# lvjiahui/DRT

Measured on AMD Instinct MI355X. Metric: M camera-rays/s (forward+backward) on 50k-tri mesh, 72 views, higher is better.
Workload: dtype f32 traversal + f64 shading/gradients; 1 GPU; horse_vh.ply x4 (1 midpoint subdivision) = 50248 tris / 25126 verts, 72 turntable views, 1024x1024 rays/view, LBVH rebuilt every step, forward+ray_loss+backward+all-reduce+SGD; targets=horse_scan.ply, mode=dropin, hip_graph=False, outputs_recycled=True, ray_binding=True, views_per_gpu=72, views_per_call=72

## Files before the change

### drt_amd/_lib.py

```python
from __future__ import annotations

import ctypes
import os

_HERE = os.path.dirname(os.path.abspath(__file__))
LIB_PATH = os.environ.get("DRT_HIP_LIB") or os.path.join(_HERE, "libdrt_hip.so")

_c = ctypes
_P = _c.c_void_p
_I64 = _c.c_int64
_D = _c.c_double

SIGNATURES = {
    "drt_last_error": (_c.c_char_p, []),
    "drt_version": (_c.c_int, []),
    "drt_deterministic": (_c.c_int, [_c.c_int]),
    "drt_fx_finalize": (_c.c_int, [_P, _I64, _P, _c.c_int, _P]),
    "drt_fx_add": (_c.c_int, [_P, _P, _I64, _P]),
    "drt_fx_to_limbs": (_c.c_int, [_P, _I64, _P, _P]),
    "drt_fx_from_limbs": (_c.c_int, [_P, _I64, _P, _P]),
    "drt_create": (_c.c_int, [_c.c_int, _c.POINTER(_P)]),
    "drt_destroy": (None, [_P]),
    "drt_update_mesh": (_c.c_int, [_P, _P, _I64, _P, _I64, _P]),
    "drt_update_vert": (_c.c_int, [_P, _P, _I64, _P]),
# ... 76 lines not shown
    "drt_rm_split_faces": (_c.c_int, [_P, _I64, _P, _P, _P, _P, _P]),
    "drt_rm_vertex_normals": (_c.c_int, [_P, _P, _P, _P, _I64, _P, _P]),
    "drt_rm_vertex_faces": (_c.c_int, [_P, _I64, _I64, _P, _P, _P, _P, _P, _P, _P]),
    "drt_rm_collapse_eval_all": (_c.c_int, [_P, _I64, _P, _P, _P, _P, _D, _D, _c.c_int, _P, _P, _P, _P, _P, _P, _P, _P, _I64, _P, _P]),
    "drt_rm_surface_filter_list": (_c.c_int, [_P, _P, _P, _P, _P, _I64, _D, _P, _P]),
    "drt_rm_surface_filter": (_c.c_int, [_P, _P, _P, _P, _I64, _c.c_int, _D, _P, _P]),
    "drt_rm_closest_near": (_c.c_int, [_P, _P, _I64, _D, _P, _P]),
    "drt_rm_kill_faces": (_c.c_int, [_P, _P, _I64, _P, _P]),
    "drt_rm_collapse_apply": (_c.c_int, [_P, _I64, _P, _P, _P, _P, _P, _P, _I64, _D, _c.c_uint32, _c.c_int, _P, _P, _P, _P, _P, _c.c_int, _P, _P, _P]),
    "drt_rm_round_end": (_c.c_int, [_P, _c.c_int, _P]),
    "drt_rm_flip_eval": (_c.c_int, [_P, _I64, _P, _P, _P, _P, _D, _P, _P, _P, _P, _P]),
    "drt_rm_flip_apply": (_c.c_int, [_I64, _P, _P, _P, _I64, _c.c_int, _P, _P, _c.c_int, _P, _P, _P]),
    "drt_rm_smooth_target": (_c.c_int, [_P, _P, _P, _P, _I64, _P, _P]),
    "drt_rm_face_agreement": (_c.c_int, [_P, _P, _P, _I64, _P, _P]),
    "drt_rm_move_check": (_c.c_int, [_P, _P, _P, _P, _P, _I64, _I64, _P, _P, _P]),
    "drt_mesh_buf_size": (_c.c_int, [_P, _c.POINTER(_I64), _c.POINTER(_I64), _P]),
    "drt_mesh_buf_copy": (_c.c_int, [_P, _P, _P]),
    "drt_mesh_buf_free": (None, [_P]),
    "drt_profile_enable": (_c.c_int, [_P, _c.c_int]),
    "drt_profile_select": (_c.c_int, [_P, _c.c_uint32]),
    "drt_profile_read": (_c.c_int, [_P, _P, _P, _P]),
    "drt_profile_trace_stats": (_c.c_int, [_P, _P]),
    "drt_route_counts": (_c.c_int, [_P, _P]),
    "drt_check_violations": (_c.c_int, [_P]),
}

_lib = None


class DrtError(RuntimeError):
    pass


def lib():
    global _lib
    if _lib is None:
        if not os.path.exists(LIB_PATH):
            raise DrtError(f"{LIB_PATH} not found: the HIP extension is not built "
                           "(run `python __graft_entry__.py`); there is no CPU fallback")
        h = ctypes.CDLL(LIB_PATH)
        for name, (res, args) in SIGNATURES.items():
            if os.environ.get("DRT_HIP_LIB") and not hasattr(h, name):
                continue
            fn = getattr(h, name)
            fn.restype = res
            fn.argtypes = args
# ... 12 lines not shown
```

### drt_amd/csrc/drt_api.hip

```cpp
#include "drt_scene.h"

static thread_local char g_err[512] = "";
int fail(int code, const char* fmt, ...) {
    va_list ap;
    va_start(ap, fmt);
    vsnprintf(g_err, sizeof(g_err), fmt, ap);
    va_end(ap);
    return code;
}

int ensure_slow_stack(drt_scene* s, hipStream_t st) {
    if (s->slow_stack) return DRT_OK;
    hipStreamCaptureStatus cap = hipStreamCaptureStatusNone;
    if (hipStreamIsCapturing(st, &cap) == hipSuccess && cap != hipStreamCaptureStatusNone)
        return fail(DRT_E_INVALID, "the first silhouette / closest-point / intersect query of a scene allocates its overflow area and cannot run inside a "
                                   "stream capture: issue one such call eagerly before capturing");
    int blocks = s->grid_trace;
    if (blocks < 4 * s->n_cu) blocks = 4 * s->n_cu;
    if (blocks < kRedoGrid) blocks = kRedoGrid;
    HIP_TRY(hipMalloc(&s->slow_stack, sizeof(int32_t) * (size_t)blocks * kTraceBlock * kStackSlowDev));
    return DRT_OK;
}

static int g_det = -1;
// ... 94 lines not shown
    if (e == hipSuccess) {
        const uint32_t init[12] = {0xFF800000u, 0xFF800000u, 0xFF800000u, 0x007FFFFFu, 0x007FFFFFu, 0x007FFFFFu,
                                   0xFF800000u, 0xFF800000u, 0xFF800000u, 0x007FFFFFu, 0x007FFFFFu, 0x007FFFFFu};
        e = hipMemcpy(s->bounds_acc, init, sizeof(init), hipMemcpyHostToDevice);
    }
    if (e == hipSuccess) e = hipMalloc(&s->vcount, sizeof(unsigned) * 4);
    if (e == hipSuccess) e = hipMemset(s->vcount, 0, sizeof(unsigned) * 4);
    if (e == hipSuccess) e = hipMalloc(&s->seg_counts, sizeof(unsigned) * drt_scene::kMaxSeg);
    if (e == hipSuccess) e = hipEventCreateWithFlags(&s->fork_ev, hipEventDisableTiming);
    if (e == hipSuccess) e = hipStreamCreateWithFlags(&s->build_stream, hipStreamNonBlocking);
    if (e == hipSuccess) e = hipEventCreateWithFlags(&s->prefill_fork, hipEventDisableTiming);
    if (e == hipSuccess) e = hipEventCreateWithFlags(&s->prefill_done, hipEventDisableTiming);
    if (e == hipSuccess) e = hipEventCreateWithFlags(&s->prefill_done_cap, hipEventDisableTiming);
    if (e == hipSuccess) e = hipEventCreateWithFlags(&s->build_fork, hipEventDisableTiming);
    if (e == hipSuccess) e = hipEventCreateWithFlags(&s->build_done, hipEventDisableTiming);
    if (const char* ev = getenv("DRT_ASYNC_BUILD")) s->async_build = atoi(ev) != 0;
    if (const char* ev = getenv("DRT_CULL_DIRECT")) s->cull_direct = atoi(ev) != 0;
    if (const char* ev = getenv("DRT_CULL_PARK")) s->cull_park = atoi(ev) != 0;
    if (const char* ev = getenv("DRT_CULL_DIRECT_MIN_LOG2")) { const int v = atoi(ev); if (v >= 0 && v <= 40) s->cull_direct_min_rays = (int64_t)1 << v; }
    if (const char* ev = getenv("DRT_TREE")) { const int v = atoi(ev); if (v >= 0 && v <= 2) s->tree_mode = v; }
    if (const char* ev = getenv("DRT_REBUILD_EVERY")) { const int v = atoi(ev); if (v >= 1) s->rebuild_every = v; }
    if (const char* ev = getenv("DRT_STREAMS")) { const int v = atoi(ev); if (v >= 1 && v <= drt_scene::kMaxSub) s->n_sub = v; }
    if (const char* ev = getenv("DRT_RASTER")) s->use_raster = atoi(ev) != 0;
    if (const char* ev = getenv("DRT_HIT_SEED")) s->hit_seed = atoi(ev) != 0;
    if (const char* ev = getenv("DRT_ARM_FINISH_BESIDE")) s->arm_finish_beside = atoi(ev) != 0;
    if (const char* ev = getenv("DRT_SEED_TILED")) s->seed_tiled = atoi(ev) != 0;
    if (const char* ev = getenv("DRT_GRID_CANARY")) s->grid_canary = atoi(ev) != 0;
    if (const char* ev = getenv("DRT_FILL_OVERLAP")) s->fill_overlap = atoi(ev) != 0;
    if (const char* ev = getenv("DRT_FILL_AFTER_SHADE1")) s->fill_after_shade1 = atoi(ev) != 0;
    if (const char* ev = getenv("DRT_SUB_PER_STREAM")) { const int v = atoi(ev); if (v >= 1 && v <= 16) s->sub_per_stream = v; }
    if (const char* ev = getenv("DRT_MIN_SUB_LOG2")) { const int v = atoi(ev); if (v >= 12 && v <= 30) s->min_sub_rays = (int64_t)1 << v; }
    for (int k = 0; k < s->n_sub && e == hipSuccess; ++k) {
        drt_scene::Sub& w = s->sub[k];
        e = hipStreamCreateWithFlags(&w.stream, hipStreamNonBlocking);
        if (e == hipSuccess) e = hipEventCreateWithFlags(&w.done, hipEventDisableTiming);
        if (e == hipSuccess) e = hipEventCreateWithFlags(&w.tail, hipEventDisableTiming);
        if (e == hipSuccess) e = hipEventCreateWithFlags(&w.fill_fork, hipEventDisableTiming);
        if (e == hipSuccess) e = hipEventCreateWithFlags(&w.fill_join, hipEventDisableTiming);
        if (e == hipSuccess) e = hipMalloc(&w.qcount, sizeof(unsigned) * kQCount);
        if (e == hipSuccess) e = hipMalloc(&w.slow_stack, sizeof(int32_t) * (size_t)kRedoGrid * kTraceBlock * kStackSlowDev);
    }
    if (e == hipSuccess) {
        hipDeviceProp_t prop;
        if (hipGetDeviceProperties(&prop, device) == hipSuccess && prop.multiProcessorCount > 0) s->n_cu = prop.multiProcessorCount;
        int per_cu;
        per_cu = query_blocks_per_cu();
// ... 18 lines not shown
        return fail(DRT_E_HIP, "hipMalloc: %s", hipGetErrorString(e));
    }
    *out = s;
    return DRT_OK;
}

void drt_destroy(drt_scene_t* s) {
    if (!s) return;
    (void)hipSetDevice(s->device);
    if (s->build_stream) (void)hipStreamSynchronize(s->build_stream);
    scene_free_mesh(s);
    if (s->build_fork) (void)hipEventDestroy(s->build_fork);
    if (s->build_done) (void)hipEventDestroy(s->build_done);
    if (s->build_stream) (void)hipStreamDestroy(s->build_stream);
    (void)hipFree(s->params);
    (void)hipFree(s->slow_stack);
    (void)hipFree(s->scratch); (void)hipFree(s->bounds_acc); (void)hipFree(s->seg_counts);
    (void)hipFree(s->b1_list); (void)hipFree(s->b1_redo); (void)hipFree(s->b1_count);
    for (int j = 0; j < drt_scene::kMaxSub; ++j) {
        drt_scene::Sub& w = s->sub[j];
        for (int k = 0; k < 3; ++k) { (void)hipFree(w.q_idx[k]); (void)hipFree(w.q_ray[k]); (void)hipFree(w.q_face[k]); }
        (void)hipFree(w.tmp_face1); (void)hipFree(w.tmp_face2); (void)hipFree(w.qcount); (void)hipFree(w.slow_stack); (void)hipFree(w.redo);
        (void)hipFree(w.zbuf); (void)hipFree(w.zmask); (void)hipFree(w.vmodel); (void)hipFree(w.big); (void)hipFree(w.big_count); (void)hipFree(w.gen_list); (void)hipFree(w.ray64);
        if (w.done) (void)hipEventDestroy(w.done);
        if (w.fill_fork) (void)hipEventDestroy(w.fill_fork);
        if (w.fill_join) (void)hipEventDestroy(w.fill_join);
        if (w.tail) (void)hipEventDestroy(w.tail);
        if (w.stream) (void)hipStreamDestroy(w.stream);
    }
    image_views_free(s);
    image_loss_free(s);
    paths_free(s);
    (void)hipFree(s->vcount);
    (void)hipFree(s->vh_list);
    if (s->fork_ev) (void)hipEventDestroy(s->fork_ev);
    if (s->prefill_fork) (void)hipEventDestroy(s->prefill_fork);
    if (s->prefill_done) (void)hipEventDestroy(s->prefill_done);
    if (s->prefill_done_cap) (void)hipEventDestroy(s->prefill_done_cap);
    for (auto& e : s->prof_ev) (void)hipEventDestroy(e);
    (void)hipFree(s->prof_counts);
    delete s;
}

int drt_profile_enable(drt_scene_t* s, int on) {
    CHECK_SCENE(s);
    if (on && s->prof_ev.empty()) {
// ... 30 lines not shown
    for (size_t k = 0; k + 1 < s->prof_used; k += 2) {
        float ms = 0.f;
        HIP_TRY(hipEventElapsedTime(&ms, s->prof_ev[k], s->prof_ev[k + 1]));
        const int stg = s->prof_stage[k / 2];
        ms_out[stg] += ms;
        launches_out[stg] += 1;
    }
    unsigned long long h[kProfStages + 12];
    HIP_TRY(hipMemcpy(h, s->prof_counts, sizeof(h), hipMemcpyDeviceToHost));
    for (int k = 0; k < kProfStages; ++k) items_out[k] = (int64_t)h[k];
    for (int k = 0; k < 12; ++k) s->trace_stats[k] = (int64_t)h[kProfStages + k];
    HIP_TRY(hipMemset(s->prof_counts, 0, sizeof(h)));
    s->prof_used = 0;
    return DRT_OK;
}

int drt_route_counts(drt_scene_t* s, int64_t* out8) {
    CHECK_SCENE(s);
    if (!out8) return fail(DRT_E_INVALID, "null pointer argument");
    for (int k = 0; k < 8; ++k) out8[k] = s->route_counts[k];
    return DRT_OK;
}

int drt_internal_stream(drt_scene_t* s, int which, void** out) {
    if (!s || !out) return fail(DRT_E_INVALID, "null pointer argument");
    if (which == 0) { *out = (void*)s->build_stream; return DRT_OK; }
    if (which >= 1 && which <= s->n_sub) { *out = (void*)s->sub[which - 1].stream; return DRT_OK; }
    return fail(DRT_E_INVALID, "no internal stream %d (0 = build, 1..%d = pipelines)", which, s->n_sub);
}

int drt_check_violations(int64_t* out4) {
    if (!out4) return fail(DRT_E_INVALID, "null pointer argument");
#if defined(DRT_CHECK)
    HIP_TRY(hipDeviceSynchronize());
    unsigned long long tot[4] = {0, 0, 0, 0};
    if (check_counters_pipeline(tot) || check_counters_trace(tot)) return fail(DRT_E_HIP, "could not read the check counters");
    for (int k = 0; k < 4; ++k) out4[k] = (int64_t)tot[k];
#else
    for (int k = 0; k < 4; ++k) out4[k] = -1;
#endif
    return DRT_OK;
}

int drt_profile_trace_stats(drt_scene_t* s, int64_t* out12) {
    CHECK_SCENE(s);
    if (!out12) return fail(DRT_E_INVALID, "null pointer argument");
// ... 7 lines not shown
```

### drt_amd/csrc/drt_build.hip

```cpp
#include "drt_device.h"
#include "drt_sort.h"
#include <algorithm>

void scene_free_mesh(drt_scene* s) {
    (void)hipFree(s->faces); (void)hipFree(s->verts); (void)hipFree(s->nodes); (void)hipFree(s->tris);
    (void)hipFree(s->keys[0]); (void)hipFree(s->keys[1]); (void)hipFree(s->idx[0]); (void)hipFree(s->idx[1]);
    (void)hipFree(s->hist); (void)hipFree(s->parent_inner); (void)hipFree(s->parent_leaf); (void)hipFree(s->flags);
    (void)hipFree(s->wide); (void)hipFree(s->range_lo); (void)hipFree(s->range_hi); (void)hipFree(s->tris_flat); (void)hipFree(s->slot_of_face);
    s->slot_of_face = nullptr; s->wide = nullptr; s->range_lo = s->range_hi = nullptr; s->tris_flat = nullptr;
    s->faces = nullptr; s->verts = nullptr; s->nodes = nullptr; s->tris = nullptr;
    s->keys[0] = s->keys[1] = s->idx[0] = s->idx[1] = nullptr;
    s->hist = nullptr; s->parent_inner = s->parent_leaf = nullptr; s->flags = nullptr;
    s->cap_faces = s->cap_verts = 0;
}

__device__ __forceinline__ uint32_t f32_ordered(float f) { const uint32_t b = __float_as_uint(f); return b ^ ((b >> 31) ? 0xFFFFFFFFu : 0x80000000u); }
__device__ __forceinline__ float f32_unordered(uint32_t u) { return __uint_as_float(u ^ ((u >> 31) ? 0x80000000u : 0xFFFFFFFFu)); }
constexpr uint32_t kOrdPosInf = 0xFF800000u, kOrdNegInf = 0x007FFFFFu;

__global__ void __launch_bounds__(256) k_cast_verts(const double* __restrict__ v64, float* __restrict__ v32, int64_t n3, uint32_t* acc,
                                                    uint32_t* __restrict__ hist_zero, int hist_entries) {
    __shared__ float red[6][4];
    for (int64_t i = blockIdx.x * (int64_t)blockDim.x + threadIdx.x; i < hist_entries; i += (int64_t)gridDim.x * blockDim.x) hist_zero[i] = 0u;
    float lo[3] = {INFINITY, INFINITY, INFINITY}, hi[3] = {-INFINITY, -INFINITY, -INFINITY};
// ... 555 lines not shown
    return DRT_OK;
}

int wait_build(drt_scene* s, hipStream_t st) {
    if (s->build_pending) HIP_TRY(hipStreamWaitEvent(st, s->build_done, 0));
    return DRT_OK;
}

extern "C" {

int drt_update_mesh(drt_scene_t* s, const int32_t* d_faces, int64_t n_faces, const float* d_verts, int64_t n_verts, void* stream) {
    CHECK_SCENE(s);
    if (n_faces < 0 || n_verts < 0 || (n_faces && !d_faces) || (n_verts && !d_verts)) return fail(DRT_E_INVALID, "bad mesh arguments");
    if (n_faces > (int64_t)1 << 30) return fail(DRT_E_INVALID, "too many faces");
    hipStream_t st = (hipStream_t)stream;
    int rc = begin_update(s, st);
    if (rc) return rc;
    if (n_faces > s->cap_faces || n_verts > s->cap_verts) HIP_TRY(hipStreamSynchronize(s->build_stream));
    rc = ensure_capacity(s, n_faces, n_verts);
    if (rc) return rc;
    s->n_faces = n_faces;
    s->n_verts = n_verts;
    s->order_valid = false;
    if (n_faces) HIP_TRY(hipMemcpyAsync(s->faces, d_faces, sizeof(int32_t) * 3 * n_faces, hipMemcpyDeviceToDevice, st));
    if (n_verts) HIP_TRY(hipMemcpyAsync(s->verts, d_verts, sizeof(float) * 3 * n_verts, hipMemcpyDeviceToDevice, st));
    s->topology_fixed = false;
    if (s->tree_mode == 2) { rc = install_sah_topology(s, st); if (rc) return rc; }
    return rebuild(s, st, nullptr);
}

int drt_update_vert(drt_scene_t* s, const float* d_verts, int64_t n_verts, void* stream) {
    CHECK_BUILT(s);
    if (n_verts != s->n_verts || (n_verts && !d_verts)) return fail(DRT_E_INVALID, "vertex count %lld != %lld", (long long)n_verts, (long long)s->n_verts);
    hipStream_t st = (hipStream_t)stream;
    int rc = begin_update(s, st);
    if (rc) return rc;
    if (n_verts) HIP_TRY(hipMemcpyAsync(s->verts, d_verts, sizeof(float) * 3 * n_verts, hipMemcpyDeviceToDevice, st));
    return rebuild(s, st, nullptr);
}

int drt_update_vert_f64(drt_scene_t* s, const double* d_verts, int64_t n_verts, void* stream) {
    CHECK_BUILT(s);
    if (n_verts != s->n_verts || (n_verts && !d_verts)) return fail(DRT_E_INVALID, "vertex count %lld != %lld", (long long)n_verts, (long long)s->n_verts);
    hipStream_t st = (hipStream_t)stream;
    int rc = begin_update(s, st);
    if (rc) return rc;
// ... 62 lines not shown
```

### drt_amd/csrc/drt_raster.h

```cpp
#pragma once
#include "drt_common.h"
#include "drt_tri.h"

namespace drt {

struct ViewModel {
    double o[3];
    double minv[9];
    int32_t ok;
    int32_t all;
};

static_assert(sizeof(ViewModel) == 104, "DRT_GRID_CACHE_BYTES of include/drt_hip.h");

constexpr double kRasterPad = 0.0625;
constexpr double kRasterVerifyTol = 1e-3;
#ifndef DRT_RASTER_MAX_PER_LANE
#define DRT_RASTER_MAX_PER_LANE 48
#endif
constexpr int kRasterMaxPerLane = DRT_RASTER_MAX_PER_LANE;
constexpr int kRasterBandPixels = 1024;

DRT_HD bool fit_view_model(d3 o, d3 d00, d3 dW0, d3 d0H, d3 dWH, double wm1, double hm1, ViewModel& vm) {
    const d3 c0 = dW0, c1 = d0H, c2 = -dWH;
// ... 52 lines not shown
    const float fx0 = fmaxf(ceilf(lox), 0.0f), fx1 = fminf(floorf(hix), (float)(w - 1));
    const float fy0 = fmaxf(ceilf(loy), 0.0f), fy1 = fminf(floorf(hiy), (float)(h - 1));
    if (fx0 > fx1 || fy0 > fy1) return r;
    r.x0 = (int)fx0; r.x1 = (int)fx1; r.y0 = (int)fy0; r.y1 = (int)fy1;
    return r;
}

DRT_HD bool tri_faces_away(f3 o32, const TriRec& t) {
    const f3 a{t.v0x - o32.x, t.v0y - o32.y, t.v0z - o32.z};
    return dot(a, cross(f3{t.e1x, t.e1y, t.e1z}, f3{t.e2x, t.e2y, t.e2z})) > 0.0f;
}

DRT_HD unsigned long long raster_key(float t, int32_t face) {
    uint32_t tb;
    memcpy(&tb, &t, 4);
    return ((unsigned long long)tb << 32) | (unsigned long long)(uint32_t)face;
}
constexpr unsigned long long kRasterEmpty = ~0ull;

DRT_HD int64_t raster_slot(unsigned x, unsigned gy, unsigned w) {
    return (((int64_t)(gy >> 2) * (w >> 2) + (x >> 2)) << 4) | ((gy & 3u) << 2) | (x & 3u);
}

}
```

### drt_amd/csrc/drt_raster.hip

```cpp
#include "drt_device.h"

__global__ void __launch_bounds__(64) k_fit_views(const double* __restrict__ origin, const double* __restrict__ dir, int w, int h,
                                                  ViewModel* __restrict__ views) {
    __shared__ ViewModel vm;
    const int64_t base = (int64_t)blockIdx.x * w * h;
    if (threadIdx.x == 0) {
        const int64_t i00 = base, iW0 = base + (w - 1), i0H = base + (int64_t)(h - 1) * w, iWH = i0H + (w - 1);
        if (fit_view_model(load_d3(origin, i00), load_d3(dir, i00), load_d3(dir, iW0), load_d3(dir, i0H), load_d3(dir, iWH),
                           (double)(w - 1), (double)(h - 1), vm))
            vm.ok = 1;
    }
    __syncthreads();
    bool good = vm.ok != 0;
    if (good) {
        const int sx = (int)(threadIdx.x & 7), sy = (int)(threadIdx.x >> 3);
        const int x = (int)(((int64_t)(w - 1) * sx) / 7), y = (int)(((int64_t)(h - 1) * sy) / 7);
        const int64_t i = base + (int64_t)y * w + x;
        good = view_verify(vm, load_d3(origin, i), load_d3(dir, i), (double)x, (double)y);
    }
    const bool all_good = __ballot(good) == ~0ull;
    if (threadIdx.x == 0) {
        vm.ok = all_good ? 1 : 0;
        vm.all = vm.ok;
        views[blockIdx.x] = vm;
// ... 52 lines not shown

__device__ __forceinline__ void raster_test(const TriRec& t, f3 o32, const double* __restrict__ dir, int64_t i, int64_t slot,
                                            unsigned long long* __restrict__ zbuf, uint32_t* __restrict__ zmask) {
    const f3 d32 = to_f32(load_d3(dir, i));
    float tt;
    if (!tri_hit_mt(o32, d32, f3{t.v0x, t.v0y, t.v0z}, f3{t.e1x, t.e1y, t.e1z}, f3{t.e2x, t.e2y, t.e2z}, tt)) return;
    const unsigned long long key = raster_key(tt, t.face);
    if (key >= zbuf[slot]) return;
    if (!hit_point_in_box(o32, d32, tt, f3{t.v0x, t.v0y, t.v0z}, f3{t.e1x, t.e1y, t.e1z}, f3{t.e2x, t.e2y, t.e2z}, t.margin)) return;
    atomicMin(&zbuf[slot], key);
    const uint32_t bit = 1u << ((i >> 6) & 31);
    if (!(zmask[i >> 11] & bit)) atomicOr(&zmask[i >> 11], bit);
}

struct BigItem { int32_t view, tri, x0, y0, nx, ny; };

struct RasterLane {
    TriRec tri;
    int32_t x0, y0, nx, end;
};

__device__ __forceinline__ float wave_uniform(float v) { return __int_as_float(__builtin_amdgcn_readfirstlane(__float_as_int(v))); }

__global__ void __launch_bounds__(256, 8) k_raster(const TriRec* __restrict__ tris, int n_tris, ViewModel* views, int n_views,
                                                   const double* __restrict__ dir, int w, int h,
                                                   unsigned long long* __restrict__ zbuf, uint32_t* __restrict__ zmask,
                                                   BigItem* __restrict__ big, unsigned* big_count, unsigned big_cap, int pass) {
    __shared__ RasterLane s_lane[256];
    const int lane = threadIdx.x & 63;
    RasterLane* const wl = s_lane + (threadIdx.x & ~63);
    const unsigned n_waves = gridDim.x * 4u, wave = __builtin_amdgcn_readfirstlane(blockIdx.x * 4u + (threadIdx.x >> 6));
    const unsigned runs_per_view = ((unsigned)n_tris + 63u) / 64u, n_runs = runs_per_view * (unsigned)n_views;
    int cur_view = -1;
    float minv32[9] = {};
    f3 o32{0.0f, 0.0f, 0.0f};
    for (unsigned run = wave; run < n_runs; run += n_waves) {
        const int view = (int)(run / runs_per_view);
        const int k = (int)(run - (unsigned)view * runs_per_view) * 64 + lane;
        if (!__hip_atomic_load(&views[view].ok, __ATOMIC_RELAXED, __HIP_MEMORY_SCOPE_AGENT)) continue;
        if (view != cur_view) {
            cur_view = view;
            for (int q = 0; q < 9; ++q) minv32[q] = wave_uniform((float)views[view].minv[q]);
            o32 = f3{wave_uniform((float)views[view].o[0]), wave_uniform((float)views[view].o[1]), wave_uniform((float)views[view].o[2])};
        }
        int count = 0;
        __builtin_amdgcn_wave_barrier();
        if (k < n_tris) {
            const TriRec tri = tris[k];
            if ((pass == 1) == tri_faces_away(o32, tri)) {
                ViewModel vm;
                for (int q = 0; q < 9; ++q) vm.minv[q] = (double)minv32[q];
                const PixelBox box = project_tri_box(vm, o32, tri, w, h);
                if (box.unsafe) {
                    __hip_atomic_store(&views[view].ok, 0, __ATOMIC_RELAXED, __HIP_MEMORY_SCOPE_AGENT);
                } else if (box.x0 <= box.x1 && box.y0 <= box.y1) {
                    const int nx = box.x1 - box.x0 + 1, ny = box.y1 - box.y0 + 1;
                    const int64_t cnt = (int64_t)nx * ny;
                    if (cnt > kRasterMaxPerLane) {
                        const int rows_per = max(1, kRasterBandPixels / nx), n_bands = (ny + rows_per - 1) / rows_per;
                        const unsigned slot = atomicAdd(big_count, (unsigned)n_bands);
                        if (slot <= big_cap && (unsigned)n_bands <= big_cap - slot) {
                            for (int b = 0; b < n_bands; ++b)
                                big[slot + b] = BigItem{view, k, box.x0, box.y0 + b * rows_per, nx, min(rows_per, ny - b * rows_per)};
                        } else {
                            __hip_atomic_store(&views[view].ok, 0, __ATOMIC_RELAXED, __HIP_MEMORY_SCOPE_AGENT);
                            for (unsigned q = slot; q < big_cap; ++q) big[q] = BigItem{view, k, 0, 0, 0, 0};
                        }
                    } else {
                        count = (int)cnt;
                        wl[lane].tri = tri;
                        wl[lane].x0 = box.x0; wl[lane].y0 = box.y0; wl[lane].nx = nx;
                    }
                }
            }
        }
        int end = count;
        for (int off = 1; off < 64; off <<= 1) {
            const int v = __shfl_up(end, off);
            if (lane >= off) end += v;
        }
        const int total = __builtin_amdgcn_readlane(end, 63);
        if (total == 0) continue;
        wl[lane].end = end;
        __builtin_amdgcn_wave_barrier();
        const int64_t base = (int64_t)view * w * h;
        for (int item0 = 0; item0 < total; item0 += 64) {
            const int item = item0 + lane;
            if (item >= total) break;
            int lo = 0, hi = 63;
            while (lo < hi) {
                const int mid = (lo + hi) >> 1;
                if (wl[mid].end > item) hi = mid; else lo = mid + 1;
            }
            const RasterLane& ow = wl[lo];
            const int local = item - (lo == 0 ? 0 : wl[lo - 1].end);
            const int row = (int)(((float)local + 0.5f) / (float)ow.nx);
            const int x = ow.x0 + (local - row * ow.nx), y = ow.y0 + row;
            raster_test(ow.tri, o32, dir, base + (int64_t)y * w + x, raster_slot((unsigned)x, (unsigned)(view * h + y), (unsigned)w), zbuf, zmask);
        }
    }
}

__global__ void __launch_bounds__(256) k_raster_big(const TriRec* __restrict__ tris, const ViewModel* __restrict__ views,
                                                    const double* __restrict__ dir, int w, int h,
                                                    unsigned long long* __restrict__ zbuf, uint32_t* __restrict__ zmask,
                                                    const BigItem* __restrict__ big, const unsigned* __restrict__ big_count, unsigned big_cap) {
    const unsigned n = min(*big_count, big_cap);
    const unsigned n_waves = gridDim.x * 4u;
    const int lane = threadIdx.x & 63;
    for (unsigned e = __builtin_amdgcn_readfirstlane(blockIdx.x * 4u + (threadIdx.x >> 6)); e < n; e += n_waves) {
        const BigItem it = big[e];
        const ViewModel& vm = views[it.view];
        const TriRec t = tris[it.tri];
        const f3 o32 = to_f32(d3{vm.o[0], vm.o[1], vm.o[2]});
        const int64_t base = (int64_t)it.view * w * h;
        const int cnt = it.nx * it.ny;
        for (int p = lane; p < cnt; p += 64) {
            const int row = (int)(((float)p + 0.5f) / (float)it.nx);
            int y = it.y0 + row, x = it.x0 + (p - row * it.nx);
            if (x >= it.x0 + it.nx) { x -= it.nx; ++y; } else if (x < it.x0) { x += it.nx; --y; }
            raster_test(t, o32, dir, base + (int64_t)y * w + x, raster_slot((unsigned)x, (unsigned)(it.view * h + y), (unsigned)w), zbuf, zmask);
        }
    }
}

__global__ void k_fill_u64(unsigned long long* __restrict__ p, int64_t n, unsigned long long v) {
    for (int64_t i = blockIdx.x * (int64_t)blockDim.x + threadIdx.x; i < n; i += (int64_t)gridDim.x * blockDim.x) p[i] = v;
}

int ensure_raster(drt_scene* s, drt_scene::Sub& w, int64_t n_rays, int n_views, hipStream_t st) {
    if (n_rays > w.z_cap) {
        (void)hipFree(w.zbuf); (void)hipFree(w.zmask);
        w.zbuf = nullptr; w.zmask = nullptr; w.z_cap = 0;
        const int64_t words = (n_rays + 2047) / 2048 + 1;
        HIP_TRY(hipMalloc(&w.zbuf, sizeof(unsigned long long) * n_rays));
        HIP_TRY(hipMalloc(&w.zmask, sizeof(uint32_t) * words));
        k_fill_u64<<<4 * s->n_cu, 256, 0, st>>>(w.zbuf, n_rays, kRasterEmpty);
        HIP_TRY(hipMemsetAsync(w.zmask, 0, sizeof(uint32_t) * words, st));
        w.z_cap = n_rays;
    }
    if (n_views > w.vm_cap) {
        (void)hipFree(w.vmodel); w.vmodel = nullptr; w.vm_cap = 0;
        HIP_TRY(hipMalloc(&w.vmodel, sizeof(ViewModel) * n_views));
        w.vm_cap = n_views;
    }
    if (!w.big) {
        HIP_TRY(hipMalloc(&w.big, sizeof(BigItem) * drt_scene::kBigCap));
        HIP_TRY(hipMalloc(&w.big_count, sizeof(unsigned)));
    }
    return DRT_OK;
}

int launch_raster(drt_scene* s, drt_scene::Sub& w, hipStream_t st, const double* d_origin, const double* d_dir, int n_views, int iw, int ih,
                  ViewModel* trusted) {
    const int n = (int)s->n_faces;
    HIP_TRY(hipMemsetAsync(w.big_count, 0, sizeof(unsigned), st));
    if (trusted) k_check_views<<<n_views, 64, 0, st>>>(d_origin, d_dir, iw, ih, trusted, w.vmodel,
                                                        s->grid_canary ? (++s->canary_salt ? s->canary_salt : ++s->canary_salt) : 0u,
                                                        s->vcount + 3);
    else k_fit_views<<<n_views, 64, 0, st>>>(d_origin, d_dir, iw, ih, w.vmodel);
    if (n > 0) {
        for (int pass = 0; pass < 2; ++pass) {
            k_raster<<<8 * s->n_cu, 256, 0, st>>>(s->tris_flat, n, w.vmodel, n_views, d_dir, iw, ih, w.zbuf, w.zmask,
                                                                      reinterpret_cast<BigItem*>(w.big), w.big_count, drt_scene::kBigCap, pass);
            if (pass == 0) {
                k_raster_big<<<8 * s->n_cu, 256, 0, st>>>(s->tris_flat, w.vmodel, d_dir, iw, ih, w.zbuf, w.zmask,
                                                           reinterpret_cast<const BigItem*>(w.big), w.big_count, drt_scene::kBigCap);
                HIP_TRY(hipMemsetAsync(w.big_count, 0, sizeof(unsigned), st));
            }
        }
        k_raster_big<<<8 * s->n_cu, 256, 0, st>>>(s->tris_flat, w.vmodel, d_dir, iw, ih, w.zbuf, w.zmask,
                                                   reinterpret_cast<const BigItem*>(w.big), w.big_count, drt_scene::kBigCap);
    }
    HIP_TRY(hipGetLastError());
    return DRT_OK;
}
```

### drt_amd/csrc/drt_scene.h

```cpp
#pragma once
#include <hip/hip_runtime.h>

#include <cstdarg>
#include <cstdio>
#include <cstdlib>
#include <cstring>
#include <new>
#include <vector>

#include "../../include/drt_hip.h"
#include "drt_common.h"
#include "drt_closest.h"
#include "drt_edge.h"
#include "drt_fixed.h"
#include "drt_lbvh.h"
#include "drt_path.h"
#include "drt_raster.h"
#include "drt_shade.h"
#include "drt_traverse.h"
#include "drt_tri.h"

using namespace drt;


// ... 72 lines not shown
    struct Sub {
        hipStream_t stream = nullptr;
        hipEvent_t done = nullptr;
        hipEvent_t tail = nullptr;
        hipEvent_t fill_fork = nullptr, fill_join = nullptr;
        int32_t* q_idx[3] = {nullptr, nullptr, nullptr};
        float* q_ray[3] = {nullptr, nullptr, nullptr};
        int32_t* q_face[3] = {nullptr, nullptr, nullptr};
        int32_t *tmp_face1 = nullptr, *tmp_face2 = nullptr;
        unsigned* qcount = nullptr;
        double* ray64 = nullptr;
        int64_t ray64_cap = 0;
        int32_t* redo = nullptr;
        int32_t* slow_stack = nullptr;
        int64_t q_cap = 0, fused_cap = 0;
        unsigned long long* zbuf = nullptr;
        uint32_t* zmask = nullptr;
        int64_t z_cap = 0;
        ViewModel* vmodel = nullptr;
        int vm_cap = 0;
        void* big = nullptr;
        unsigned* big_count = nullptr;
        int32_t* gen_list = nullptr;
    };
    static constexpr unsigned kBigCap = 1u << 20;
    static constexpr int kMaxSub = 4;
    Sub sub[kMaxSub];
    int n_sub = 2;
    int sub_per_stream = 1;
    int64_t min_sub_rays = 1 << 24;
    hipEvent_t fork_ev = nullptr;
    struct Clean { double* ori = nullptr; double* dir = nullptr; uint8_t* mask = nullptr; int64_t n = 0; const int32_t* rows = nullptr; const int64_t* n_rows = nullptr;
                   bool captured = false;  } clean;
    static constexpr int kMaxSeg = 32;
    unsigned* seg_counts = nullptr;
    struct Segs { const int32_t* list = nullptr; int n = 0; int stream0 = 0; } segs;
    struct Prefill { const void* ptr = nullptr; int64_t bytes = 0; };
    Prefill prefill[3];
    int n_prefill = 0;
    hipEvent_t prefill_fork = nullptr, prefill_done = nullptr, prefill_done_cap = nullptr;
    unsigned* vcount = nullptr;
    uint32_t* vh_list = nullptr;
    int64_t vh_cap = 0;
    bool prof_on = false;
    uint32_t prof_mask = ~0u;
    bool prof_stats = false;
// ... 4 lines not shown
    size_t prof_dropped = 0;
    unsigned long long* prof_counts = nullptr;
    hipStream_t prof_stream = nullptr;
    int n_cu = 256;
    int grid_trace = 2048;
    int grid_path = 2048;
    int64_t trace_stats[12] = {0};
    int grid_mega = 1024;
    int64_t mega_max_rays = 0;
    int shade_min = 8;
    int mega_refill_min = 16;
    int refill_min = 32;
    int inner_min = 24;
    int64_t chunk_rays = kChunkRays;

    bool fill_after_shade1 = true;
    bool fill_overlap = true;
    bool grid_canary = true;
    unsigned canary_salt = 0;
    bool seed_tiled = true;
    bool arm_finish_beside = true;
    bool hit_seed = true;
    bool use_raster = true;
    bool built = false;
    void* paths_ws = nullptr;
    void* image_loss_ws = nullptr;
    void* image_views = nullptr;
};


int query_blocks_per_cu();
int pipeline_blocks_per_cu();
int mega_blocks_per_cu();

int ensure_raster(drt_scene* s, drt_scene::Sub& w, int64_t n_rays, int n_views, hipStream_t st);
int launch_raster(drt_scene* s, drt_scene::Sub& w, hipStream_t st, const double* d_origin, const double* d_dir, int n_views, int iw, int ih,
                  ViewModel* trusted);

void paths_free(drt_scene* s);
void image_loss_free(drt_scene* s);
void image_views_free(drt_scene* s);

int ensure_slow_stack(drt_scene* s, hipStream_t st);
bool det_mode();
#define DET_LAUNCH(kern, grid, block, st, ...)                                        \
    do {                                                                              \
// ... 66 lines not shown
```

### drt_amd/optix_mesh.py

```python
from __future__ import annotations

import ctypes

import torch

from . import _lib


_raw_stream = getattr(torch._C, "_cuda_getCurrentRawStream", None)
_raw_device = getattr(torch._C, "_cuda_getDevice", None)


def _stream():
    if _raw_stream is not None and _raw_device is not None:
        return ctypes.c_void_p(_raw_stream(_raw_device()))
    return ctypes.c_void_p(torch.cuda.current_stream().cuda_stream)


class _NoContext:
    def __enter__(self):
        return None

    def __exit__(self, *exc):
        return False
# ... 144 lines not shown
        with _on(self.device):
            _lib.check(_lib.lib().drt_profile_enable(self._h, int(on)))

    def profile_select(self, stages=None):
        mask = 0xFFFFFFFF if stages is None else sum(1 << self.STAGES.index(k) for k in stages)
        _lib.check(_lib.lib().drt_profile_select(self._h, mask))

    def profile_read(self):
        n = len(self.STAGES)
        ms = (ctypes.c_double * n)()
        launches = (ctypes.c_int64 * n)()
        items = (ctypes.c_int64 * n)()
        with _on(self.device):
            _lib.check(_lib.lib().drt_profile_read(self._h, ms, launches, items))
        return {k: (ms[i], launches[i], items[i]) for i, k in enumerate(self.STAGES)}

    ROUTES = ("total", "raster", "trust", "direct", "park", "late_fill", "tree_late", "mega")

    def route_counts(self):
        out = (ctypes.c_int64 * len(self.ROUTES))()
        _lib.check(_lib.lib().drt_route_counts(self._h, out))
        return dict(zip(self.ROUTES, out))

    def trace_stats(self):
        out = (ctypes.c_int64 * 12)()
        _lib.check(_lib.lib().drt_profile_trace_stats(self._h, out))
        return {f"trace{k + 1}": tuple(out[4 * k:4 * k + 4]) for k in range(3)}
```

### include/drt_hip.h

```cpp
#ifndef DRT_HIP_H
#define DRT_HIP_H

#include <stdint.h>

#ifdef __cplusplus
extern "C" {
#endif

#define DRT_OK            0
#define DRT_E_INVALID    -1
#define DRT_E_HIP        -2
#define DRT_E_NOMEM      -3

typedef struct drt_scene drt_scene_t;

const char* drt_last_error(void);
int drt_version(void);

#define DRT_FX_BYTES_PER_VALUE 24
int drt_deterministic(int on);
int drt_fx_finalize(const void* d_cells, int64_t n, double* d_out, int accumulate, void* stream);
int drt_fx_add(void* d_dst_cells, const void* d_src_cells, int64_t n, void* stream);
int drt_fx_to_limbs(const void* d_cells, int64_t n, int64_t* d_limbs, void* stream);
int drt_fx_from_limbs(const int64_t* d_limbs, int64_t n, void* d_cells, void* stream);
// ... 269 lines not shown
                            const float* d_texture, int tex_h, int tex_w, int channels, const double* fill_void, const double* fill_invalid,
                            float* d_image, float* d_hit, float* d_through, const double* sigma, float* d_length, void* stream);
int drt_render_image_loss_absorb(drt_scene_t* s, const double* d_verts, const double* camera21, int height, int width, int y0, int y1, int supersample,
                                 double ior_int, double ior_ext, int max_bounces, int law_flags, int fresnel, const double* screen9,
                                 const float* d_texture, int tex_h, int tex_w, int channels, const double* fill_void, const double* fill_invalid,
                                 const float* d_target, const float* d_weight, double* d_loss, double* d_grad_verts, double* d_grad_ior, float* d_image,
                                 int64_t* d_count, const double* sigma, double* d_grad_sigma, void* stream);

typedef struct drt_image_views drt_image_views_t;
int drt_image_views_check(int n_views, const double* cameras21, const double* screens9, int height, int width);
int drt_image_views_create(drt_scene_t* s, int n_views, const double* cameras21, const double* screens9, int height, int width, drt_image_views_t** out);
void drt_image_views_destroy(drt_image_views_t* views);
int drt_render_image_loss_views(drt_scene_t* s, const double* d_verts, const drt_image_views_t* views, const int* view_ids, int k, int r0, int r1,
                                int supersample, double ior_int, double ior_ext, int max_bounces, int law_flags, int fresnel, const float* d_texture,
                                int tex_h, int tex_w, int channels, const double* fill_void, const double* fill_invalid, const float* d_targets,
                                const float* d_weights, double* d_loss, double* d_grad_verts, double* d_grad_ior, int64_t* d_count, void* stream);

#define DRT_PROFILE_STAGES 14
int drt_profile_enable(drt_scene_t* s, int on);
int drt_profile_select(drt_scene_t* s, uint32_t stage_mask);
int drt_profile_read(drt_scene_t* s, double* ms_out, int64_t* launches_out, int64_t* items_out);
int drt_profile_trace_stats(drt_scene_t* s, int64_t* out12);
int drt_route_counts(drt_scene_t* s, int64_t* out8);

int drt_check_violations(int64_t* out4);

#ifdef __cplusplus
}
#endif
#endif
```

Before: 45250 M camera-rays/s.

## Balance raster work across waves using per-run cost recorded on previous call

The raster kernel now records per-run pixel-work counts, and a new prefix-sum kernel builds a table that splits the total weighted work evenly across waves. On the next call with matching views and geometry, each wave processes a contiguous range of runs, including partial runs at the boundaries, instead of strided runs. This targets load imbalance from uneven triangle footprints. It adds a record store per run, an extra deal kernel launch, and relies on costs from the previous step, which can be stale after vertex updates.

Result: faster. 46710 M camera-rays/s (median of 6 runs) (+3.2%).

```diff
diff --git a/drt_amd/_lib.py b/drt_amd/_lib.py
--- a/drt_amd/_lib.py
+++ b/drt_amd/_lib.py
@@ -122,6 +122,7 @@
     "drt_profile_read": (_c.c_int, [_P, _P, _P, _P]),
     "drt_profile_trace_stats": (_c.c_int, [_P, _P]),
     "drt_route_counts": (_c.c_int, [_P, _P]),
+    "drt_raster_deal_counts": (_c.c_int, [_P, _P]),
     "drt_check_violations": (_c.c_int, [_P]),
 }
 
diff --git a/drt_amd/csrc/drt_api.hip b/drt_amd/csrc/drt_api.hip
--- a/drt_amd/csrc/drt_api.hip
+++ b/drt_amd/csrc/drt_api.hip
@@ -140,6 +140,9 @@
     if (const char* ev = getenv("DRT_REBUILD_EVERY")) { const int v = atoi(ev); if (v >= 1) s->rebuild_every = v; }
     if (const char* ev = getenv("DRT_STREAMS")) { const int v = atoi(ev); if (v >= 1 && v <= drt_scene::kMaxSub) s->n_sub = v; }
     if (const char* ev = getenv("DRT_RASTER")) s->use_raster = atoi(ev) != 0;
+    if (const char* ev = getenv("DRT_RASTER_DEAL")) s->raster_deal = atoi(ev) != 0;
+    if (const char* ev = getenv("DRT_RASTER_DEAL_MIN_RUNS")) { const long long v = atoll(ev); if (v >= 0) s->raster_deal_min_runs = v; }
+    if (const char* ev = getenv("DRT_RASTER_DEAL_FIXED")) { const int v = atoi(ev); if (v >= 1 && v <= 65536) s->raster_deal_fixed = (uint32_t)v; }
     if (const char* ev = getenv("DRT_HIT_SEED")) s->hit_seed = atoi(ev) != 0;
     if (const char* ev = getenv("DRT_ARM_FINISH_BESIDE")) s->arm_finish_beside = atoi(ev) != 0;
     if (const char* ev = getenv("DRT_SEED_TILED")) s->seed_tiled = atoi(ev) != 0;
@@ -204,6 +207,7 @@
         for (int k = 0; k < 3; ++k) { (void)hipFree(w.q_idx[k]); (void)hipFree(w.q_ray[k]); (void)hipFree(w.q_face[k]); }
         (void)hipFree(w.tmp_face1); (void)hipFree(w.tmp_face2); (void)hipFree(w.qcount); (void)hipFree(w.slow_stack); (void)hipFree(w.redo);
         (void)hipFree(w.zbuf); (void)hipFree(w.zmask); (void)hipFree(w.vmodel); (void)hipFree(w.big); (void)hipFree(w.big_count); (void)hipFree(w.gen_list); (void)hipFree(w.ray64);
+        (void)hipFree(w.deal.table);
         if (w.done) (void)hipEventDestroy(w.done);
         if (w.fill_fork) (void)hipEventDestroy(w.fill_fork);
         if (w.fill_join) (void)hipEventDestroy(w.fill_join);
@@ -280,6 +284,13 @@
     return DRT_OK;
 }
 
+int drt_raster_deal_counts(drt_scene_t* s, int64_t* out2) {
+    CHECK_SCENE(s);
+    if (!out2) return fail(DRT_E_INVALID, "null pointer argument");
+    out2[0] = s->raster_deal_counts[0]; out2[1] = s->raster_deal_counts[1];
+    return DRT_OK;
+}
+
 int drt_internal_stream(drt_scene_t* s, int which, void** out) {
     if (!s || !out) return fail(DRT_E_INVALID, "null pointer argument");
     if (which == 0) { *out = (void*)s->build_stream; return DRT_OK; }
diff --git a/drt_amd/csrc/drt_build.hip b/drt_amd/csrc/drt_build.hip
--- a/drt_amd/csrc/drt_build.hip
+++ b/drt_amd/csrc/drt_build.hip
@@ -601,6 +601,7 @@
     s->n_faces = n_faces;
     s->n_verts = n_verts;
     s->order_valid = false;
+    for (int j = 0; j < drt_scene::kMaxSub; ++j) s->sub[j].deal.complete = false;
     if (n_faces) HIP_TRY(hipMemcpyAsync(s->faces, d_faces, sizeof(int32_t) * 3 * n_faces, hipMemcpyDeviceToDevice, st));
     if (n_verts) HIP_TRY(hipMemcpyAsync(s->verts, d_verts, sizeof(float) * 3 * n_verts, hipMemcpyDeviceToDevice, st));
     s->topology_fixed = false;
diff --git a/drt_amd/csrc/drt_raster.h b/drt_amd/csrc/drt_raster.h
--- a/drt_amd/csrc/drt_raster.h
+++ b/drt_amd/csrc/drt_raster.h
@@ -98,4 +98,59 @@
     return (((int64_t)(gy >> 2) * (w >> 2) + (x >> 2)) << 4) | ((gy & 3u) << 2) | (x & 3u);
 }
 
+struct DealPos { uint32_t run, item; };
+constexpr uint32_t kRasterDealFixed = 64;
+
+DRT_HD uint64_t raster_deal_weight(uint32_t cost, uint32_t c_fixed) { return (uint64_t)c_fixed + cost; }
+DRT_HD uint64_t raster_deal_target(uint64_t total, uint32_t n_waves, uint32_t v) {
+    return (total / n_waves) * v + (total % n_waves) * v / n_waves;
 }
+DRT_HD uint32_t raster_deal_item(uint64_t off, uint32_t c_fixed) { return off > c_fixed ? (uint32_t)(off - c_fixed) : 0u; }
+
+DRT_HD DealPos raster_deal_boundary(const uint64_t* prefix, uint32_t n_runs, uint32_t n_waves, uint32_t v, uint32_t c_fixed) {
+    if (v == 0 || n_runs == 0) return DealPos{0, 0};
+    if (v >= n_waves) return DealPos{n_runs, 0};
+    const uint64_t total = prefix[n_runs - 1];
+    const uint64_t target = raster_deal_target(total, n_waves, v);
+    uint32_t lo = 0, hi = n_runs - 1;
+    while (lo < hi) {
+        const uint32_t mid = lo + ((hi - lo) >> 1);
+        if (prefix[mid] > target) hi = mid; else lo = mid + 1;
+    }
+    return DealPos{lo, raster_deal_item(target - (lo ? prefix[lo - 1] : 0), c_fixed)};
+}
+
+DRT_HD uint32_t raster_deal_first_wave(uint64_t sum, uint64_t total, uint32_t n_waves) {
+    const uint64_t q = (sum * n_waves + total - 1) / total;
+    return q > n_waves ? n_waves : (uint32_t)q;
+}
+DRT_HD void raster_deal_place(DealPos* table, uint32_t run, uint64_t before, uint64_t with, uint64_t total, uint32_t n_waves, uint32_t c_fixed) {
+    if (!(with > before) || total == 0) return;
+    const uint32_t v1 = raster_deal_first_wave(with, total, n_waves);
+    for (uint32_t v = raster_deal_first_wave(before, total, n_waves); v < v1; ++v)
+        table[v] = DealPos{run, raster_deal_item(raster_deal_target(total, n_waves, v) - before, c_fixed)};
+}
+
+DRT_HD DealPos raster_deal_clamp(DealPos b, uint32_t n_runs) { return b.run >= n_runs ? DealPos{n_runs, 0} : b; }
+
+DRT_HD uint32_t raster_deal_end(DealPos b0, DealPos b1) {
+    if (b0.run == b1.run && b0.item == b1.item) return b0.run;
+    return b1.run + (b1.item > 0 ? 1u : 0u);
+}
+
+struct DealSlice { uint32_t lo, hi; bool owner; };
+DRT_HD DealSlice raster_deal_slice(DealPos b0, DealPos b1, uint32_t r) {
+    DealSlice s;
+    s.lo = b0.run == r ? b0.item : 0u;
+    s.hi = b1.run == r ? b1.item : 0xFFFFFFFFu;
+    s.owner = (b0.run < r || (b0.run == r && b0.item == 0)) && (r < b1.run || (r == b1.run && b1.item > 0));
+    return s;
+}
+
+
+struct DealRange { uint32_t run, end, lo, last_hi; };
+DRT_HD DealRange raster_deal_range(DealPos b0, DealPos b1) { return DealRange{b0.run, raster_deal_end(b0, b1), b0.item, b1.item ? b1.item : 0xFFFFFFFFu}; }
+DRT_HD DealSlice raster_deal_slice(const DealRange& g) { return DealSlice{g.lo, g.run + 1 == g.end ? g.last_hi : 0xFFFFFFFFu, g.lo == 0}; }
+DRT_HD void raster_deal_next(DealRange& g) { ++g.run; g.lo = 0; }
+
+}
diff --git a/drt_amd/csrc/drt_raster.hip b/drt_amd/csrc/drt_raster.hip
--- a/drt_amd/csrc/drt_raster.hip
+++ b/drt_amd/csrc/drt_raster.hip
@@ -98,10 +98,14 @@
 
 __device__ __forceinline__ float wave_uniform(float v) { return __int_as_float(__builtin_amdgcn_readfirstlane(__float_as_int(v))); }
 
+constexpr int kRasterCostAt = 32;
+template <bool DEAL, bool RECORD, int pass>
 __global__ void __launch_bounds__(256, 8) k_raster(const TriRec* __restrict__ tris, int n_tris, ViewModel* views, int n_views,
                                                    const double* __restrict__ dir, int w, int h,
                                                    unsigned long long* __restrict__ zbuf, uint32_t* __restrict__ zmask,
-                                                   BigItem* __restrict__ big, unsigned* big_count, unsigned big_cap, int pass) {
+                                                   BigItem* __restrict__ big, unsigned* big_count,
+                                                   const DealPos* __restrict__ table ) {
+    constexpr unsigned big_cap = drt_scene::kBigCap;
     __shared__ RasterLane s_lane[256];
     const int lane = threadIdx.x & 63;
     RasterLane* const wl = s_lane + (threadIdx.x & ~63);
@@ -110,32 +114,43 @@
     int cur_view = -1;
     float minv32[9] = {};
     f3 o32{0.0f, 0.0f, 0.0f};
-    for (unsigned run = wave; run < n_runs; run += n_waves) {
+    DealRange g{wave, n_runs, 0u, 0xFFFFFFFFu};
+    if (DEAL) {
+        const DealPos b0 = wave == 0 ? DealPos{0, 0} : raster_deal_clamp(table[wave], n_runs);
+        const DealPos b1 = wave + 1 >= n_waves ? DealPos{n_runs, 0} : raster_deal_clamp(table[wave + 1], n_runs);
+        g = raster_deal_range(b0, b1);
+        g.end = min(g.end, n_runs);
+    }
+    for (; g.run < g.end; DEAL ? raster_deal_next(g) : (void)(g.run += n_waves)) {
+        const unsigned run = g.run;
         const int view = (int)(run / runs_per_view);
         const int k = (int)(run - (unsigned)view * runs_per_view) * 64 + lane;
-        if (!__hip_atomic_load(&views[view].ok, __ATOMIC_RELAXED, __HIP_MEMORY_SCOPE_AGENT)) continue;
-        if (view != cur_view) {
+        const DealSlice sl = DEAL ? raster_deal_slice(g) : DealSlice{0u, 0xFFFFFFFFu, true};
+        const bool ok = __hip_atomic_load(&views[view].ok, __ATOMIC_RELAXED, __HIP_MEMORY_SCOPE_AGENT) != 0;
+        if (!RECORD && !ok) continue;
+        if (ok && view != cur_view) {
             cur_view = view;
             for (int q = 0; q < 9; ++q) minv32[q] = wave_uniform((float)views[view].minv[q]);
             o32 = f3{wave_uniform((float)views[view].o[0]), wave_uniform((float)views[view].o[1]), wave_uniform((float)views[view].o[2])};
         }
         int count = 0;
         __builtin_amdgcn_wave_barrier();
-        if (k < n_tris) {
+        if ((!RECORD || ok) && k < n_tris) {
             const TriRec tri = tris[k];
             if ((pass == 1) == tri_faces_away(o32, tri)) {
                 ViewModel vm;
                 for (int q = 0; q < 9; ++q) vm.minv[q] = (double)minv32[q];
                 const PixelBox box = project_tri_box(vm, o32, tri, w, h);
                 if (box.unsafe) {
-                    __hip_atomic_store(&views[view].ok, 0, __ATOMIC_RELAXED, __HIP_MEMORY_SCOPE_AGENT);
+                    if (sl.owner) __hip_atomic_store(&views[view].ok, 0, __ATOMIC_RELAXED, __HIP_MEMORY_SCOPE_AGENT);
                 } else if (box.x0 <= box.x1 && box.y0 <= box.y1) {
                     const int nx = box.x1 - box.x0 + 1, ny = box.y1 - box.y0 + 1;
                     const int64_t cnt = (int64_t)nx * ny;
                     if (cnt > kRasterMaxPerLane) {
                         const int rows_per = max(1, kRasterBandPixels / nx), n_bands = (ny + rows_per - 1) / rows_per;
-                        const unsigned slot = atomicAdd(big_count, (unsigned)n_bands);
-                        if (slot <= big_cap && (unsigned)n_bands <= big_cap - slot) {
+                        const unsigned slot = sl.owner ? atomicAdd(big_count, (unsigned)n_bands) : 0u;
+                        if (!sl.owner) {
+                        } else if (slot <= big_cap && (unsigned)n_bands <= big_cap - slot) {
                             for (int b = 0; b < n_bands; ++b)
                                 big[slot + b] = BigItem{view, k, box.x0, box.y0 + b * rows_per, nx, min(rows_per, ny - b * rows_per)};
                         } else {
@@ -156,13 +171,15 @@
             if (lane >= off) end += v;
         }
         const int total = __builtin_amdgcn_readlane(end, 63);
-        if (total == 0) continue;
+        if (RECORD && sl.owner && lane == 0) big_count[kRasterCostAt + 2 * run + pass] = (unsigned)total;
+        const int stop = (int)min((unsigned)total, sl.hi);
+        if (sl.lo >= (unsigned)stop) continue;
         wl[lane].end = end;
         __builtin_amdgcn_wave_barrier();
         const int64_t base = (int64_t)view * w * h;
-        for (int item0 = 0; item0 < total; item0 += 64) {
+        for (int item0 = (int)sl.lo; item0 < stop; item0 += 64) {
             const int item = item0 + lane;
-            if (item >= total) break;
+            if (item >= stop) break;
             int lo = 0, hi = 63;
             while (lo < hi) {
                 const int mid = (lo + hi) >> 1;
@@ -175,6 +192,44 @@
             raster_test(ow.tri, o32, dir, base + (int64_t)y * w + x, raster_slot((unsigned)x, (unsigned)(view * h + y), (unsigned)w), zbuf, zmask);
         }
     }
+}
+
+constexpr int kDealBlock = 1024;
+__device__ __forceinline__ uint64_t shfl_up_u64(uint64_t v, int off) {
+    return ((uint64_t)(uint32_t)__shfl_up((int)(v >> 32), off) << 32) | (uint32_t)__shfl_up((int)(uint32_t)v, off);
+}
+__global__ void __launch_bounds__(kDealBlock) k_raster_deal(const unsigned* __restrict__ counts , DealPos* __restrict__ table,
+                                                            unsigned n_runs, unsigned n_waves, uint32_t c_fixed) {
+    __shared__ uint64_t s_all[kDealBlock / 64], s_before[kDealBlock / 64], s_own[kDealBlock / 64];
+    const unsigned pass = blockIdx.y, tid = threadIdx.x, lane = tid & 63, wid = tid >> 6;
+    DealPos* const tab = table + pass * (n_waves + 1);
+    const unsigned* const cost = counts + kRasterCostAt + pass;
+    const unsigned first = blockIdx.x * kDealBlock, run = first + tid;
+    constexpr unsigned kMost = 64u * (unsigned)kRasterMaxPerLane;
+    uint64_t all = 0, before = 0, own = 0;
+    for (unsigned base = 0; base < n_runs; base += kDealBlock) {
+        const unsigned r = base + tid;
+        const uint64_t wgt = r < n_runs ? raster_deal_weight(min(cost[2 * r], kMost), c_fixed) : 0;
+        all += wgt;
+        if (base < first) before += wgt;
+        if (base == first) own = wgt;
+    }
+    uint64_t incl = own;
+    for (int off = 1; off < 64; off <<= 1) {
+        const uint64_t v = shfl_up_u64(incl, off), va = shfl_up_u64(all, off), vb = shfl_up_u64(before, off);
+        if ((int)lane >= off) { incl += v; all += va; before += vb; }
+    }
+    if (lane == 63) { s_all[wid] = all; s_before[wid] = before; s_own[wid] = incl; }
+    __syncthreads();
+    uint64_t total = 0, start = 0;
+    for (unsigned q = 0; q < kDealBlock / 64; ++q) {
+        total += s_all[q];
+        start += s_before[q];
+        if (q < wid) start += s_own[q];
+    }
+    const uint64_t with = start + incl;
+    if (run < n_runs) raster_deal_place(tab, run, with - own, with, total, n_waves, c_fixed);
+    if (run == 0) tab[n_waves] = DealPos{n_runs, 0};
 }
 
 __global__ void __launch_bounds__(256) k_raster_big(const TriRec* __restrict__ tris, const ViewModel* __restrict__ views,
@@ -204,6 +259,9 @@
     for (int64_t i = blockIdx.x * (int64_t)blockDim.x + threadIdx.x; i < n; i += (int64_t)gridDim.x * blockDim.x) p[i] = v;
 }
 
+constexpr int64_t kRasterDealMaxRuns = (int64_t)1 << 18;
+static int64_t raster_runs(int64_t n_tris, int n_views) { return (n_tris + 63) / 64 * n_views; }
+
 int ensure_raster(drt_scene* s, drt_scene::Sub& w, int64_t n_rays, int n_views, hipStream_t st) {
     if (n_rays > w.z_cap) {
         (void)hipFree(w.zbuf); (void)hipFree(w.zmask);
@@ -220,9 +278,15 @@
         HIP_TRY(hipMalloc(&w.vmodel, sizeof(ViewModel) * n_views));
         w.vm_cap = n_views;
     }
-    if (!w.big) {
-        HIP_TRY(hipMalloc(&w.big, sizeof(BigItem) * drt_scene::kBigCap));
-        HIP_TRY(hipMalloc(&w.big_count, sizeof(unsigned)));
+    if (!w.big) HIP_TRY(hipMalloc(&w.big, sizeof(BigItem) * drt_scene::kBigCap));
+    drt_scene::Sub::Deal& dl = w.deal;
+    if (!w.big_count) {
+        const int n_waves = 8 * s->n_cu * 4;
+        HIP_TRY(hipMalloc(&w.big_count, sizeof(unsigned) * (kRasterCostAt + (s->raster_deal ? 2 * kRasterDealMaxRuns : 0))));
+        if (s->raster_deal) {
+            HIP_TRY(hipMalloc(&dl.table, sizeof(DealPos) * 2 * (n_waves + 1)));
+            dl.cap_runs = kRasterDealMaxRuns; dl.cap_waves = n_waves;
+        }
     }
     return DRT_OK;
 }
@@ -236,9 +300,17 @@
                                                         s->vcount + 3);
     else k_fit_views<<<n_views, 64, 0, st>>>(d_origin, d_dir, iw, ih, w.vmodel);
     if (n > 0) {
+        drt_scene::Sub::Deal& dl = w.deal;
+        const int grid = 8 * s->n_cu;
+        const int64_t n_runs = raster_runs(n, n_views);
+        const bool record = s->raster_deal && dl.table && n_runs > 0 && n_runs >= s->raster_deal_min_runs && n_runs <= dl.cap_runs && grid * 4 == dl.cap_waves;
+        const bool dealt = record && dl.complete && dl.dir == d_dir && dl.n_views == n_views && dl.iw == iw && dl.ih == ih && dl.n_tris == n && dl.grid == grid;
+        s->raster_deal_counts[dealt ? 0 : 1] += 2;
         for (int pass = 0; pass < 2; ++pass) {
-            k_raster<<<8 * s->n_cu, 256, 0, st>>>(s->tris_flat, n, w.vmodel, n_views, d_dir, iw, ih, w.zbuf, w.zmask,
-                                                                      reinterpret_cast<BigItem*>(w.big), w.big_count, drt_scene::kBigCap, pass);
+            auto* const kern = pass == 0 ? (dealt ? k_raster<true, true, 0> : record ? k_raster<false, true, 0> : k_raster<false, false, 0>)
+                                         : (dealt ? k_raster<true, true, 1> : record ? k_raster<false, true, 1> : k_raster<false, false, 1>);
+            kern<<<grid, 256, 0, st>>>(s->tris_flat, n, w.vmodel, n_views, d_dir, iw, ih, w.zbuf, w.zmask, reinterpret_cast<BigItem*>(w.big), w.big_count,
+                                       dealt ? dl.table + pass * (dl.cap_waves + 1) : nullptr);
             if (pass == 0) {
                 k_raster_big<<<8 * s->n_cu, 256, 0, st>>>(s->tris_flat, w.vmodel, d_dir, iw, ih, w.zbuf, w.zmask,
                                                            reinterpret_cast<const BigItem*>(w.big), w.big_count, drt_scene::kBigCap);
@@ -247,6 +319,12 @@
         }
         k_raster_big<<<8 * s->n_cu, 256, 0, st>>>(s->tris_flat, w.vmodel, d_dir, iw, ih, w.zbuf, w.zmask,
                                                    reinterpret_cast<const BigItem*>(w.big), w.big_count, drt_scene::kBigCap);
+        dl.complete = false;
+        if (record) {
+            k_raster_deal<<<dim3((unsigned)((n_runs + kDealBlock - 1) / kDealBlock), 2), kDealBlock, 0, st>>>(w.big_count, dl.table, (unsigned)n_runs, (unsigned)(grid * 4), s->raster_deal_fixed);
+            dl.dir = d_dir; dl.n_views = n_views; dl.iw = iw; dl.ih = ih; dl.n_tris = n; dl.grid = grid;
+            dl.complete = true;
+        }
     }
     HIP_TRY(hipGetLastError());
     return DRT_OK;
diff --git a/drt_amd/csrc/drt_scene.h b/drt_amd/csrc/drt_scene.h
--- a/drt_amd/csrc/drt_scene.h
+++ b/drt_amd/csrc/drt_scene.h
@@ -118,6 +118,14 @@
         void* big = nullptr;
         unsigned* big_count = nullptr;
         int32_t* gen_list = nullptr;
+        struct Deal {
+            DealPos* table = nullptr;
+            int64_t cap_runs = 0;
+            int cap_waves = 0;
+            const double* dir = nullptr;
+            int n_views = 0, iw = 0, ih = 0, n_tris = 0, grid = 0;
+            bool complete = false;
+        } deal;
     };
     static constexpr unsigned kBigCap = 1u << 20;
     static constexpr int kMaxSub = 4;
@@ -168,6 +176,10 @@
     bool arm_finish_beside = true;
     bool hit_seed = true;
     bool use_raster = true;
+    bool raster_deal = true;
+    int64_t raster_deal_min_runs = 16384;
+    uint32_t raster_deal_fixed = kRasterDealFixed;
+    int64_t raster_deal_counts[2] = {0, 0};
     bool built = false;
     void* paths_ws = nullptr;
     void* image_loss_ws = nullptr;
diff --git a/drt_amd/optix_mesh.py b/drt_amd/optix_mesh.py
--- a/drt_amd/optix_mesh.py
+++ b/drt_amd/optix_mesh.py
@@ -190,6 +190,11 @@
         _lib.check(_lib.lib().drt_route_counts(self._h, out))
         return dict(zip(self.ROUTES, out))
 
+    def raster_deal_counts(self):
+        out = (ctypes.c_int64 * 2)()
+        _lib.check(_lib.lib().drt_raster_deal_counts(self._h, out))
+        return tuple(out)
+
     def trace_stats(self):
         out = (ctypes.c_int64 * 12)()
         _lib.check(_lib.lib().drt_profile_trace_stats(self._h, out))
diff --git a/include/drt_hip.h b/include/drt_hip.h
--- a/include/drt_hip.h
+++ b/include/drt_hip.h
@@ -315,6 +315,7 @@
 int drt_profile_read(drt_scene_t* s, double* ms_out, int64_t* launches_out, int64_t* items_out);
 int drt_profile_trace_stats(drt_scene_t* s, int64_t* out12);
 int drt_route_counts(drt_scene_t* s, int64_t* out8);
+int drt_raster_deal_counts(drt_scene_t* s, int64_t* out2);
 
 int drt_check_violations(int64_t* out4);
 
```
